# ekzhang/rpt

Measured on AMD Instinct MI355X. Metric: Msamples/s, higher is better.
Workload: dtype f64

## Files before the change

rpt_amd/csrc/api_render.cpp:

```cpp
#include "api_internal.h"

namespace rptapi {

int event_pair_begin(rptgpu_scene* h, int kind, bool on) {
  h->stats.kernel_launches[kind]++;
  if (!on || h->ev_used + 2 > MAX_EVENT_PAIRS * 2) return -1;
  while ((int)h->ev_pool.size() < h->ev_used + 2) {
    hipEvent_t e;
    HIP_TRY(hipEventCreate(&e));
    h->ev_pool.push_back(e);
  }
  const int e0 = h->ev_used;
  h->ev_used += 2;
  HIP_TRY(hipEventRecord(h->ev_pool[e0], h->stream));
  return e0;
}
void event_pair_end(rptgpu_scene* h, int kind, int e0) {
  if (e0 < 0) return;
  HIP_TRY(hipEventRecord(h->ev_pool[e0 + 1], h->stream));
  h->pending.push_back({kind, e0, e0 + 1});
}

struct Bracket {
  rptgpu_scene* h;
// ... 219 lines not shown
  tree_query(h, kt, ps, nullptr, n, -1, nullptr, nullptr, hook);
}
void query_visibility(rptgpu_scene* h, const KernelTable* kt, const rptdev::PathState& ps, int l, uint32_t n,
                      const uint32_t* d_n, const QueryHook* hook) {
  tree_query(h, kt, ps, h->shadow_q.p + (uint64_t)l * ps.cap, n, l, h->srt.p, d_n, hook);
}

rptdev::Camera make_camera(const RptCamera& c) {
  rptdev::Camera d{};
  std::memcpy(d.eye, c.eye, sizeof d.eye);
  std::memcpy(d.direction, c.direction, sizeof d.direction);
  std::memcpy(d.up, c.up, sizeof d.up);
  d.d = 1.0 / std::tan(c.fov / 2.0);
  const double* a = c.direction;
  const double* b = c.up;
  double cr[3] = {a[1] * b[2] - a[2] * b[1], a[2] * b[0] - a[0] * b[2], a[0] * b[1] - a[1] * b[0]};
  double len = std::sqrt((cr[0] * cr[0] + cr[1] * cr[1]) + cr[2] * cr[2]);
  for (int k = 0; k < 3; k++) d.right[k] = cr[k] / len;
  d.aperture = c.aperture;
  d.focal_distance = c.focal_distance;
  return d;
}

const char* bad_params(const RptRenderParams* p) {
  if (!p->width || !p->height || !p->iterations) return "width, height and iterations must be non-zero";
  if (p->max_bounces > 254) return "max_bounces > 254";
  if ((uint64_t)p->width * p->height >= (1ull << 31)) return "frame too large";
  if (p->part_count && p->part_index >= p->part_count) return "part_index >= part_count";
  if (p->precision_mode != RPT_PRECISION_F64_STRICT) return BAD_MODE;
  return nullptr;
}

int64_t free_memory() {
  size_t free_b = 0, total_b = 0;
  return hipMemGetInfo(&free_b, &total_b) == hipSuccess ? (int64_t)free_b : -1;
}

rptdev::PathState path_state(rptgpu_scene* h) {
  rptdev::PathState ps{};
  ps.ray = h->ray.p; ps.hit = h->hit.p; ps.hit_obj = h->hit_obj.p; ps.draw = h->draw.p;
  ps.pid = h->pid.p; ps.col = h->col.p;
  ps.ray_next = h->ray_next.p; ps.draw_next = h->draw_next.p; ps.pid_next = h->pid_next.p; ps.col_next = h->col_next.p;
  ps.rec = h->rec.p; ps.rec_parent = h->rec_parent.p; ps.last_col = h->last_col.p;
  ps.shadow = h->shadow.p; ps.cap = h->ws_cap; ps.rec_cap = h->ws_rec_cols;
  if (h->path_reorder) {
    ps.sort_keys = h->sort_kin.p; ps.sort_vals = h->sort_vin.p; ps.next_rows = h->next_rows.p;
    std::memcpy(ps.key_bounds, h->scene_bounds, sizeof ps.key_bounds);
  }
  return ps;
}

void render_persistent(rptgpu_scene* h, const KernelTable* kt, const RptRenderParams& p, rptdev::Frame fr,
                       const rptdev::Camera& cam, void* out, bool out_f32, bool packed, bool prof) {
  hipStream_t st = h->stream;
  const uint32_t npix = fr.npix;
  const bool print_launch = std::getenv("RPTGPU_PRINT_LAUNCH") != nullptr;
  const uint64_t lbuf_held = h->lbuf.n * sizeof(double);
  const int64_t free_b = lbuf_held < h->lbuf_max_bytes ? free_memory() : -1;
  const bool flat = h->all_flat && !h->dscene.force_general;
  FlatLayout lay = flat ? h->flat_layout : FlatLayout{};
  const uint32_t flat_lds = lay.off_end;
  if (RPT_PRETRACE_CULL && lay.pretrace_cull) {
    for (size_t i = 0; i < h->obj_geom.size() && i < 64 && lay.cull_n < (uint32_t)RPT_CULL_MAX; i++) {
      uint32_t r[4];
      if (((lay.cull_always >> i) & 1ull) ||
          !rpthost::pinhole_screen_rect(rpthost::world_box(h->obj_geom[i], h->top_insts[i]), cam, fr.width, fr.height, r))
        continue;
      lay.cull_obj[lay.cull_n] = (uint32_t)i;
      const bool off = r[0] > r[1] || r[2] > r[3];
      lay.cull_lo[lay.cull_n] = off ? 0xffffffffu : (r[0] | (r[2] << 16));
      lay.cull_ext[lay.cull_n] = off ? 0u : ((r[1] - r[0]) | ((r[3] - r[2]) << 16));
      lay.cull_n++;
    }
  }
  const rptplan::PersistentPlan pl = rptplan::plan_persistent(
      npix, p.iterations, p.max_bounces, h->num_cus, kt->paths_max_blocks_per_cu(flat ? &lay : nullptr, flat_lds, false),
      h->lbuf_max_bytes, lbuf_held, free_b, h->paths_chunk, h->all_flat, h->dscene.force_general, h->flat_layout.obj_filter);
  bool park = flat && h->opt.env_park != 0 && h->dscene.env_kind != RPT_ENV_COLOR;
  if (park && kt->paths_max_blocks_per_cu(&lay, flat_lds, true) < pl.per_cu) park = false;
  h->prec.alloc((uint64_t)rpt_fold_ring_slots(p.max_bounces) * rptdev::REC_FIELDS * ((uint64_t)pl.nblocks * 64));
  h->lbuf.alloc(std::max<uint64_t>(1, (uint64_t)pl.spp_l * 3 * npix));
  if (print_launch)
    std::fprintf(stderr, "rpt_paths<%s>: %d blocks/CU x %d CUs -> %u blocks, %u samples per work item, %u launch(es) of %u spp, "
                 "dynamic LDS %u B per wave (the flat scene's tables)%s%s%s\n",
                 flat ? (lay.obj_filter ? "KdFlatF" : lay.n_tris ? "KdFlat" : "KdFlatG") : "KdLds", pl.per_cu, h->num_cus, pl.nblocks,
                 pl.chunk, pl.n_launch, pl.spp_l, flat_lds, park ? " + parked environment lookups" : "",
                 flat && lay.n_tris && lay.fuse_query && !park ? ", shadow and bounce rays in one query" : "",
                 flat && lay.n_tris && lay.fuse_query && !park && lay.scene_consts ? ", a hit's scene constants from the wave's tables" : "");
  h->counters.alloc(4);
  h->pcounters.alloc(16);
  HIP_TRY(hipMemsetAsync(h->pcounters.p, 0, 16 * sizeof(unsigned long long), st));
  for (uint32_t s0 = 0; s0 < p.iterations; s0 += pl.spp_l) {
    const uint32_t spp = std::min(pl.spp_l, p.iterations - s0);
    const uint64_t items = rptplan::work_items(npix, spp, pl.chunk);
    fr.sample_base = p.sample_index_base + s0;
    HIP_TRY(hipMemsetAsync(h->counters.p, 0, sizeof(uint32_t), st));
    { Bracket b(h, RPT_K_PATHS, prof);
      kt->paths(st, h->dscene, fr, cam, h->counters.p, h->prec.p, h->pcounters.p, h->lbuf.p, spp, pl.chunk, (uint32_t)items,
                pl.nblocks, lay, flat, flat_lds, park, h->opt.paths_batch);
      b.done(); }
    kt->sum_samples(st, fr, h->lbuf.p, spp, s0 == 0);
    if (print_launch) {
      uint32_t ended = 0;
      HIP_TRY(hipMemcpyAsync(&ended, h->counters.p, sizeof ended, hipMemcpyDeviceToHost, st));
      HIP_TRY(hipStreamSynchronize(st));
      const uint32_t batch_used = h->opt.paths_batch ? std::min<uint32_t>(h->opt.paths_batch, RPT_PATHS_BATCH_MAX)
                                                      : std::min(256u, std::max((uint32_t)items / (std::max(1u, pl.nblocks) * 32u), 16u));
      std::fprintf(stderr, "rpt_paths work counter: ended at %u for %llu items; %u waves, claims of at most %u: dead claims %lld of at most %llu\n",
                   ended, (unsigned long long)items, pl.nblocks, batch_used, (long long)ended - (long long)items,
                   (unsigned long long)pl.nblocks * (64u + batch_used));
    }
  }
  HIP_TRY(hipGetLastError());
  kt->finish(st, fr, (double)p.iterations, std::pow(2.0, p.exposure_value), out, out_f32, packed);
  unsigned long long rc[16] = {0};
  HIP_TRY(hipMemcpyAsync(rc, h->pcounters.p, sizeof rc, hipMemcpyDeviceToHost, st));
  HIP_TRY(hipStreamSynchronize(st));
  if (std::getenv("RPTGPU_PRINT_PHASES")) print_prof(kt, "rpt_paths");
  h->stats.samples += (uint64_t)npix * p.iterations;
  h->stats.extend_rays += rc[0];
  h->stats.shadow_rays += rc[1];
  h->stats.shadow_rays_traced += rc[1];
}

bool run_pass(rptgpu_scene* h, const KernelTable* kt, const RptRenderParams& p, const rptdev::Frame& fr,
              const RaySource& src, uint32_t n_paths, uint32_t spp, bool prof, const QueryHook& qhook, uint64_t* cols) {
  hipStream_t st = h->stream;
  rptdev::PathState ps = path_state(h);
  const int nlights = h->dscene.num_lights;
  const uint32_t nctr = 2u + (uint32_t)nlights;
  HIP_TRY(hipMemsetAsync(h->counters.p, 0, 2 * (size_t)nctr * sizeof(uint32_t), st));
  uint32_t cset = 0;
  if (h->has_deep) reset_tree_counters(h);
  { Bracket b(h, RPT_K_RAYGEN, prof);
    if (src.cam) kt->raygen(st, fr, *src.cam, ps, n_paths);
    else kt->raygen_rays(st, fr, src.origins, src.dirs, src.first_draw, src.ids_out, src.id_base, ps, n_paths);
    b.done(); }
  h->stats.samples += n_paths;
  uint32_t n_active = n_paths;
  const uint32_t* const queue = nullptr;
  uint32_t* const next = nullptr;
  uint64_t rec_off = 0;
  const bool by_object = h->has_deep && (!(p.flags & RPT_FLAG_GENERAL_TRAVERSAL) || h->tree_kids);
  for (uint32_t depth = 0; depth <= p.max_bounces && n_active; depth++) {
    if (rec_off + n_active > h->ws_rec_cols) {
      *cols = rec_off + n_active;
      return false;
    }
    { Bracket b(h, RPT_K_EXTEND, prof);
      if (by_object)
        query_closest(h, kt, ps, n_active, &qhook);
      else
        kt->extend(st, h->dscene, ps, queue, n_active);
      b.done(); }
    h->stats.extend_rays += n_active;
    uint32_t* const ctrs = h->counters.p + (size_t)cset * nctr;
    uint32_t* const ctrs_next = h->counters.p + (size_t)(cset ^ 1u) * nctr;
    cset ^= 1u;
    { Bracket b(h, RPT_K_SHADE, prof);
      kt->shade(st, h->dscene, fr, ps, queue, n_active, depth, next, ctrs, h->shadow_q.p, ctrs_next, nctr, (uint32_t)rec_off); b.done(); }
    h->cnt_host.resize(2 + (size_t)nlights);
    uint32_t* cnt = h->cnt_host.data();
    HIP_TRY(hipMemcpyAsync(cnt, ctrs, (2 + (size_t)nlights) * sizeof(uint32_t), hipMemcpyDeviceToHost, st));
    HIP_TRY(hipStreamSynchronize(st));
    for (int l = 0; l < nlights; l++) h->stats.shadow_rays_traced += cnt[2 + l];
    if (prof && h->pending.size() >= 256) drain_events(h);
    h->stats.shadow_rays += (uint64_t)cnt[1] * (uint64_t)h->dscene.num_shadow_lights;
    if (nlights > 0) {
      Bracket b(h, RPT_K_SHADOW, prof);
      if (by_object) {
        for (int l = 0; l < nlights; l++)
// ... 226 lines not shown
```

rpt_amd/csrc/kernels.h:

```cpp
#pragma once
#include <hip/hip_runtime.h>
#include <stdint.h>

#include "device_types.h"
#include "launch_limits.h"

#ifndef RPT_FLAT_RUN
#define RPT_FLAT_RUN 6
#endif

#define RPT_PATHS_WAVE_LDS 20480u
#define RPT_PATHS_WALKER_LDS 2560u
#ifndef RPT_RAY_STASH
#define RPT_RAY_STASH 2
#endif
#ifndef RPT_FUSE_QUERY
#define RPT_FUSE_QUERY 1
#endif
#ifndef RPT_SHADE_SPLIT
#define RPT_SHADE_SPLIT 1
#endif
#ifndef RPT_PRETRACE_CULL
#define RPT_PRETRACE_CULL 1
#endif
#define RPT_CULL_MAX 4
#ifndef RPT_SCENE_CONSTS
#define RPT_SCENE_CONSTS 5
#endif
#define RPT_MAT_CONSTS_BYTES 88u
#define RPT_CUBE_NORMALS_BYTES 144u
#define RPT_PATHS_STASH_LDS 4864u
#define RPT_PATHS_STASH_HIT_LDS 6656u
#define RPT_PATHS_STASH_MAX_LDS (RPT_RAY_STASH >= 2 ? RPT_PATHS_STASH_HIT_LDS : RPT_PATHS_STASH_LDS)
#ifndef RPT_PARK_K
#define RPT_PARK_K 4
#endif
#define RPT_PATHS_PARK_LDS (RPT_PARK_K * 2624u)
#ifndef RPT_PATH_REORDER_MIN
#define RPT_PATH_REORDER_MIN (1u << 20)
#endif

#define RPT_RETIRE_ITEMS 16u
#define RPT_RETIRE_TILE (RPT_RETIRE_ITEMS * 256u)

struct FlatLayout {
  uint32_t off_tris, off_refs, off_mat, off_leaf;
  uint32_t off_end;
  uint32_t n_refs, n_tris;
  uint32_t off_qtab, plane_cnt;
  const double* plane_vals;
  uint32_t obj_filter;
  uint32_t off_obox;
  const rptdev::LeafBox* obj_box;
  const double* obj_grid;
  uint64_t obj_always;
  uint32_t fuse_query;
  uint32_t pretrace_cull, cull_n;
  uint64_t cull_always;
  uint32_t cull_obj[RPT_CULL_MAX], cull_lo[RPT_CULL_MAX], cull_ext[RPT_CULL_MAX];
  uint32_t scene_consts, off_consts;
};

struct SortBufs {
  uint32_t *keys_in, *keys_out, *vals_in;
  void* tmp;
  size_t tmp_bytes;
};

#ifndef RPT_TT_WAVES
#define RPT_TT_WAVES 4
#endif
#ifndef RPT_TT_LEVELS
#define RPT_TT_LEVELS 7
#endif
#define RPT_TT_LEVELS_MIN RPT_TT_LEVELS
struct GenericStack {
  double* defer;
  double* frame;
  uint32_t threads, levels, frames;
};
struct StackSpill {
  uint32_t* node;
  double* ts;
  double* bmax;
  uint32_t threads;
  uint32_t zeros_common;
  double* rays;
  GenericStack gen;
  uint32_t* gen_overflow;
  uint32_t gen_blocks_few, gen_blocks_all;
};

struct QueryHook {
  void (*mark)(void* ctx, int kind, int end);
  void* ctx;
};

struct QueryTuning {
  uint32_t ctr_set;
  uint32_t sort_min_rays;
};

struct KernelTable {
  void (*raygen)(hipStream_t, const rptdev::Frame&, const rptdev::Camera&, const rptdev::PathState&, uint32_t n_paths);
  void (*raygen_rays)(hipStream_t, const rptdev::Frame&, const double* origins, const double* dirs, uint32_t first_draw,
                      uint32_t* ids_out, uint32_t id_base, const rptdev::PathState&, uint32_t n_paths);
  void (*extend)(hipStream_t, const rptdev::Scene&, const rptdev::PathState&, const uint32_t* queue, uint32_t n);
  void (*extend_rays)(hipStream_t, const rptdev::Scene&, const double* o, const double* d, uint64_t n, double* out_t,
                      double* out_n, int32_t* out_obj);
  void (*shade)(hipStream_t, const rptdev::Scene&, const rptdev::Frame&, const rptdev::PathState&,
                const uint32_t* queue, uint32_t n, uint32_t depth, uint32_t* next_queue, uint32_t* counters, uint32_t* sq,
                uint32_t* zero_next , uint32_t zero_n,
                uint32_t rec_off );
  void (*shadow_rays)(hipStream_t, const rptdev::Scene&, const rptdev::PathState&, const uint32_t* sq_all,
                      const uint32_t* sq_counts, uint32_t n_max, int num_lights, double* srt);
// ... 44 lines not shown
```

rpt_amd/csrc/kernels/paths.inc:

```

#ifndef RPT_PARK_FLUSH
#define RPT_PARK_FLUSH 160
#endif
struct ParkLds {
  double d[RPT_PARK_K][3][64];
  uint32_t u[RPT_PARK_K][4][64];
  uint8_t list[RPT_PARK_K * 64];
};
static_assert(sizeof(ParkLds) == RPT_PATHS_PARK_LDS, "kernels.h sizes the wave's LDS budget with it");
static_assert(RPT_PARK_K >= 1 && RPT_PARK_K <= 4, "two bits for the entry in ParkLds::list, three for a lane's count");
struct PersistArgs {
  uint32_t* work_counter;
  double* rec;
  unsigned long long* ray_counters;
  double* lbuf;
  uint32_t spp;
  uint32_t chunk;
  uint32_t n_items;
  uint32_t nthreads;
  uint32_t ring;
  uint32_t batch;
  uint32_t park_off;
  FlatLayout flat;
};
// ... 73 lines not shown
}
RPT_DEV void path_ended(const PersistArgs& pa, const Frame& fr, double* __restrict__ rec, double (*fold_l)[64],
                        uint32_t (*fold_u)[64], uint32_t lane, uint32_t& fold_st, const D3& A, uint32_t depth, uint32_t b,
                        uint32_t s, uint32_t p_local) {
  if (depth == 0) {
    double* lb = pa.lbuf + (uint64_t)s * 3 * fr.npix + p_local;
    lb[0] = A.x;
    lb[fr.npix] = A.y;
    lb[2 * (uint64_t)fr.npix] = A.z;
  } else if ((fold_st & 0xffffu) == 0u) {
    fold_l[0][lane] = A.x; fold_l[1][lane] = A.y; fold_l[2][lane] = A.z;
    fold_u[0][lane] = depth; fold_u[1][lane] = b; fold_u[2][lane] = s; fold_u[3][lane] = p_local;
    fold_st |= depth;
  } else {
    double* r = rec + b * REC_FIELDS;
    r[0] = A.x; r[1] = A.y; r[2] = A.z;
    r[3] = __longlong_as_double((long long)((uint64_t)s | ((uint64_t)p_local << 32)));
    r[4] = __longlong_as_double((long long)depth);
  }
}
RPT_DEV void park_push(ParkLds& park, uint32_t lane, uint32_t& pcnt, uint32_t& park_hd, uint32_t& park_recs, uint32_t& fold_st,
                       uint32_t ring, const D3& d, uint32_t depth, uint32_t s, uint32_t p_local) {
  const uint32_t k = pcnt, b = fold_st >> 16;
  park.d[k][0][lane] = d.x; park.d[k][1][lane] = d.y; park.d[k][2][lane] = d.z;
  park.u[k][0][lane] = depth; park.u[k][1][lane] = b; park.u[k][2][lane] = s; park.u[k][3][lane] = p_local;
  if (depth != 0u) {
    if (park_hd == 0xffffffffu) park_hd = b;
    park_recs += depth;
    fold_st = (fold_st & 0xffffu) | (next_header_slot(b, depth, ring) << 16);
  }
  pcnt = k + 1u;
}
struct RayStash {
  double v[7][64];
  uint32_t u[5][64];
};
static_assert(sizeof(RayStash) == RPT_PATHS_STASH_LDS, "kernels.h sizes the wave's LDS budget with it");
struct RayStashHit {
  double v[10][64];
  uint32_t u[6][64];
};
static_assert(sizeof(RayStashHit) == RPT_PATHS_STASH_HIT_LDS, "kernels.h sizes the wave's LDS budget with it");
template <class S> RPT_DEV void stash_put_pos(S& st, uint32_t lane, const D3& o) {
  st.v[0][lane] = o.x; st.v[1][lane] = o.y; st.v[2][lane] = o.z;
}
template <class S> RPT_DEV void stash_put_dir(S& st, uint32_t lane, const D3& d) {
  st.v[3][lane] = d.x; st.v[4][lane] = d.y; st.v[5][lane] = d.z;
}
template <class S> RPT_DEV void stash_put_ray(S& st, uint32_t lane, const D3& o, const D3& d) {
  stash_put_pos(st, lane, o);
  stash_put_dir(st, lane, d);
}
template <class S> RPT_DEV void stash_take_ray(const S& st, uint32_t lane, D3& o, D3& d) {
  o = mk(st.v[0][lane], st.v[1][lane], st.v[2][lane]);
  d = mk(st.v[3][lane], st.v[4][lane], st.v[5][lane]);
}
template <class S> RPT_DEV void stash_swap_ray(S& st, uint32_t lane, D3& o, D3& d) {
  D3 so, sd;
  stash_take_ray(st, lane, so, sd);
  stash_put_ray(st, lane, o, d);
  o = so; d = sd;
}
template <class S> RPT_DEV void stash_put_path(S& st, uint32_t lane, uint32_t p_local, uint32_t pixel, uint32_t s, uint32_t s_end, const Rng& r) {
  st.v[6][lane] = __longlong_as_double((long long)r.hi);
  st.u[0][lane] = p_local; st.u[1][lane] = pixel; st.u[2][lane] = s; st.u[3][lane] = s_end;
  st.u[4][lane] = r.draw;
}
template <class S> RPT_DEV void stash_take_path(const S& st, uint32_t lane, const Frame& fr, uint32_t& p_local, uint32_t& pixel, uint32_t& s,
                             uint32_t& s_end, Rng& r) {
  p_local = st.u[0][lane]; pixel = st.u[1][lane]; s = st.u[2][lane]; s_end = st.u[3][lane];
  r = rng_make(fr.seed, pixel, fr.sample_base + s, 0);
  r.draw = st.u[4][lane];
  r.hi = (uint64_t)__double_as_longlong(st.v[6][lane]);
}
RPT_DEV void stash_put_hit(RayStashHit& st, uint32_t lane, const D3& pos, const D3& nrm, int obj) {
  stash_put_pos(st, lane, pos);
  st.v[7][lane] = nrm.x; st.v[8][lane] = nrm.y; st.v[9][lane] = nrm.z;
  st.u[5][lane] = (uint32_t)obj;
}
RPT_DEV void stash_take_hit(const RayStashHit& st, uint32_t lane, D3& pos, D3& d, D3& nrm, int& obj) {
  stash_take_ray(st, lane, pos, d);
  nrm = mk(st.v[7][lane], st.v[8][lane], st.v[9][lane]);
  obj = (int)st.u[5][lane];
}
#ifndef RPT_STASH_REFILL_MIN
#define RPT_STASH_REFILL_MIN 32
#endif
RPT_DEV void end_path(const PersistArgs& pa, const Frame& fr, double* __restrict__ rec, double (*fold_l)[64],
                      uint32_t (*fold_u)[64], uint32_t lane, uint32_t& fold_st, uint32_t ring, const D3& A, uint32_t depth,
                      uint32_t s, uint32_t p_local) {
  const uint32_t b = fold_st >> 16;
  path_ended(pa, fr, rec, fold_l, fold_u, lane, fold_st, A, depth, b, s, p_local);
  if (depth != 0u) fold_st = (fold_st & 0xffffu) | (next_header_slot(b, depth, ring) << 16);
}
template <bool PARK>
RPT_DEV void walker_step(const PersistArgs& pa, const Frame& fr, const double* __restrict__ rec, double (*fold_l)[64],
                         uint32_t (*fold_u)[64], uint32_t lane, uint32_t& fold_st, uint32_t ring, uint32_t park_hd,
                         double probe_chk ) {
  const uint32_t wk = fold_st & 0xffffu, cb = fold_st >> 16;
  const uint32_t wD = fold_u[0][lane], wb = fold_u[1][lane];
  uint32_t pos = wb + wk;
  if (pos >= ring) pos -= ring;
  const uint32_t nh = next_header_slot(wb, wD, ring);
  const bool last = wk == 1u, more = last && nh != cb && (!PARK || nh != park_hd);
  double v[REC_FIELDS], hd[5] = {0.0, 0.0, 0.0, 0.0, 0.0};
#ifdef RPT_PROBE_NO_RING
  (void)pos;
#pragma unroll
  for (int q = 0; q < REC_FIELDS; q++) v[q] = probe_chk * (double)(q + 1);
#else
  {
    const double* r = rec + pos * REC_FIELDS;
#pragma unroll
    for (int q = 0; q < REC_FIELDS; q++) v[q] = r[q];
  }
#endif
  if (more) {
    const double* r = rec + nh * REC_FIELDS;
#pragma unroll
    for (int q = 0; q < 5; q++) hd[q] = r[q];
  }
  D3 L = mk(fold_l[0][lane], fold_l[1][lane], fold_l[2][lane]);
  D3 Ak = mk(v[0], v[1], v[2]);
  D3 f = mk(v[3], v[4], v[5]);
  D3 indirect = v[6] * cmul(f, L) * v[7];
  L = mk(Ak.x + fmin(indirect.x, FIREFLY_CLAMP), Ak.y + fmin(indirect.y, FIREFLY_CLAMP),
         Ak.z + fmin(indirect.z, FIREFLY_CLAMP));
  if (!last) {
    fold_l[0][lane] = L.x; fold_l[1][lane] = L.y; fold_l[2][lane] = L.z;
    fold_st -= 1u;
  } else {
    double* lb = pa.lbuf + (uint64_t)fold_u[2][lane] * 3 * fr.npix + fold_u[3][lane];
    lb[0] = L.x;
    lb[fr.npix] = L.y;
    lb[2 * (uint64_t)fr.npix] = L.z;
    uint32_t nk = 0u;
    if (more) {
      const uint64_t sp = (uint64_t)__double_as_longlong(hd[3]);
      nk = (uint32_t)__double_as_longlong(hd[4]);
      fold_l[0][lane] = hd[0]; fold_l[1][lane] = hd[1]; fold_l[2][lane] = hd[2];
      fold_u[0][lane] = nk; fold_u[1][lane] = nh; fold_u[2][lane] = (uint32_t)sp; fold_u[3][lane] = (uint32_t)(sp >> 32);
    }
    fold_st = (cb << 16) | nk;
  }
}
template <class LDS, bool PARK ,
          bool FUSE = false ,
          bool CONSTS = false >
__global__ void __launch_bounds__(64, RPT_PATHS_WAVES) rpt_paths(Scene sc, Frame fr, Camera cam, PersistArgs pa) {
  extern __shared__ __attribute__((aligned(16))) unsigned char flat_smem[];
  __shared__ typename PathsLds<LDS>::type kd_store;
  LDS* kd_ldsp = reinterpret_cast<LDS*>(&kd_store);
  constexpr bool FILTERED = std::is_same<LDS, KdFlatF>::value;
  constexpr bool IS_FLAT = std::is_same<LDS, KdFlat>::value || std::is_same<LDS, KdFlatG>::value || FILTERED;
  constexpr bool TRIS_IN_LDS = std::is_same<LDS, KdFlat>::value;
  FlatLds fl{};
  if constexpr (IS_FLAT) {
    const FlatLayout& lay = pa.flat;
    const uint32_t l = threadIdx.x;
    TriX* l_lrec = reinterpret_cast<TriX*>(flat_smem);
    Tri* l_tris = reinterpret_cast<Tri*>(flat_smem + lay.off_tris);
    uint32_t* l_refs = reinterpret_cast<uint32_t*>(flat_smem + lay.off_refs);
    Material* l_mat = reinterpret_cast<Material*>(flat_smem + lay.off_mat);
    uint32_t(*l_leaf)[4] = reinterpret_cast<uint32_t(*)[4]>(flat_smem + lay.off_leaf);
    const double* src = reinterpret_cast<const double*>(sc.lrec);
    double* dst = reinterpret_cast<double*>(l_lrec);
    for (uint32_t i = l; i < lay.n_refs * (uint32_t)(sizeof(TriX) / 8); i += 64) dst[i] = src[i];
    if constexpr (TRIS_IN_LDS) {
      src = reinterpret_cast<const double*>(sc.tris);
      dst = reinterpret_cast<double*>(l_tris);
      for (uint32_t i = l; i < lay.n_tris * (uint32_t)(sizeof(Tri) / 8); i += 64) dst[i] = src[i];
    }
    for (uint32_t i = l; i < lay.n_refs; i += 64) l_refs[i] = sc.refs[i];
    for (uint32_t i = l; i < (uint32_t)sc.num_objects * (uint32_t)(sizeof(Material) / 8); i += 64) {
      uint32_t ob = i / (uint32_t)(sizeof(Material) / 8), w = i - ob * (uint32_t)(sizeof(Material) / 8);
      reinterpret_cast<double*>(l_mat)[i] = reinterpret_cast<const double*>(sc.materials + sc.insts[ob].material)[w];
    }
    for (uint32_t ob = l; ob < (uint32_t)sc.num_objects; ob += 64) {
      const Inst& in = sc.insts[ob];
      uint32_t e0 = 0, e1 = 0, e2 = 0, e3 = 0;
      if (in.kind == RPT_SHAPE_MESH) {
        const Tree& tr = sc.trees[in.tree];
        e0 = tr.ref_base; e1 = tr.prim_base; e2 = tr.root_first; e3 = tr.root_leaf - 1u;
      }
      l_leaf[ob][0] = e0; l_leaf[ob][1] = e1; l_leaf[ob][2] = e2; l_leaf[ob][3] = e3;
      if constexpr (FILTERED) {
        l_leaf[ob][3] = e3 | ((uint32_t)in.kind << 8) | (in.has_xf ? 1u << 16 : 0u);
        double* ob6 = reinterpret_cast<double*>(flat_smem + lay.off_obox) + 6u * ob;
        for (int k = 0; k < 6; k++) ob6[k] = in.bounds[k];
      }
    }
    if constexpr (CONSTS) {
      static_assert(FUSE, "the tables serve the fused form");
      scene_consts_fill(sc, sc.tris, l, flat_smem + lay.off_consts);
      fl.consts = flat_smem + lay.off_consts;
    }
    __syncthreads();
    sc.lrec = l_lrec;
    if constexpr (TRIS_IN_LDS) sc.tris = l_tris;
    sc.refs = l_refs;
    fl.lrec = l_lrec; fl.tris = sc.tris; fl.refs = l_refs; fl.obj_mat = l_mat; fl.obj_leaf = l_leaf;
    fl.qtab = reinterpret_cast<double*>(flat_smem + lay.off_qtab);
    fl.plane_vals = lay.plane_vals;
    fl.plane_cnt = lay.plane_cnt;
    if constexpr (FILTERED) {
      fl.obox = reinterpret_cast<const double*>(flat_smem + lay.off_obox);
      fl.obj_box = lay.obj_box; fl.obj_grid = lay.obj_grid; fl.obj_always = lay.obj_always;
    }
  }
  const uint32_t tid = blockIdx.x * blockDim.x + threadIdx.x;
  const uint32_t lane = __lane_id();
  double* __restrict__ rec = pa.rec + (uint64_t)tid * pa.ring * REC_FIELDS;
  __shared__ double fold_l[3][64];
  __shared__ uint32_t fold_u[4][64];
  uint32_t fold_st = 0;
  const uint32_t ring = pa.ring;
  uint32_t p_local = 0, pixel = 0, s = 0, s_end = 0, depth = 0;
  bool done = false, in_path = false;
  D3 o = mk(0, 0, 0), d = mk(0, 0, 1);
  Rng rng = rng_make(fr.seed, 0, 0, 0);
  uint32_t n_ext = 0, n_sh = 0;
#ifdef RPT_PROBE_NO_RING
  double probe_chk = 0.0;
#else
  constexpr double probe_chk = 0.0;
#endif
  const double dim = (double)max(fr.width, fr.height);
  constexpr bool STASH = RPT_RAY_STASH && std::is_same<LDS, KdFlat>::value;
  constexpr bool PRETRACE = STASH && RPT_RAY_STASH >= 2 && !PARK;
  static_assert(!FUSE || PRETRACE, "the fused form is a form of the pre-traced kernel");
  using StashT = typename std::conditional<PRETRACE, RayStashHit, RayStash>::type;
  __shared__ typename std::conditional<STASH, StashT, int>::type stash_store;
  auto& stash = *reinterpret_cast<StashT*>(&stash_store);
  bool stash_valid = false, exhausted = false;
  bool pend = false;
#if RPT_PRETRACE_CULL
  uint32_t near = ~0u;
#endif
  ItemPool pool{0u, 0u, 0u};
  constexpr bool park_on = PARK;
  ParkLds& park = *reinterpret_cast<ParkLds*>(flat_smem + (park_on ? pa.park_off : 0u));
  uint32_t pcnt = 0, park_hd = 0xffffffffu, park_recs = 0;
  D3 nx_pos = mk(0, 0, 0), nx_nrm = mk(0, 0, 0);
  int nx_obj = -1;
  PROF_INIT();

  for (;;) {
    if constexpr (STASH) {
      bool refill = __ballot(!in_path && !stash_valid && !exhausted) != 0ull;
      if constexpr (PRETRACE) refill = refill || __popcll(__ballot(!stash_valid && !exhausted)) >= RPT_STASH_REFILL_MIN;
      if (refill) {
        const bool gen = !stash_valid && !exhausted;
        uint32_t g_p_local = p_local, g_pixel = pixel, g_s = s + (in_path ? 1u : 0u), g_s_end = s_end;
        const bool want_item = gen && g_s >= g_s_end;
        const bool got = fetch_item(pa, fr, lane, want_item, pool, g_p_local, g_pixel, g_s, g_s_end);
        if (want_item && !got) exhausted = true;
        PROF_PHASE(PF_P_FETCH);
        if (gen && !exhausted) {
          D3 go, gd;
          Rng gr;
          camera_ray(fr, cam, dim, g_pixel, g_s, go, gd, gr);
#if RPT_PRETRACE_CULL
          if constexpr (FUSE) near = cull_near(pa.flat, g_pixel, fr.width);
#endif
          stash_put_ray(stash, lane, go, gd);
          stash_put_path(stash, lane, g_p_local, g_pixel, g_s, g_s_end, gr);
          stash_valid = true;
          pend = PRETRACE;
        }
        PROF_PHASE(PF_P_RAYGEN);
      }
      if (!PRETRACE && !in_path && stash_valid) {
        stash_take_ray(stash, lane, o, d);
        stash_take_path(stash, lane, fr, p_local, pixel, s, s_end, rng);
        stash_valid = false;
        depth = 0;
        in_path = true;
      }
      done = !in_path && exhausted && !(PRETRACE && stash_valid);
      if (__ballot(!done || (fold_st & 0xffffu) != 0u || pcnt != 0u) == 0) break;
    } else {
      const bool need = !done && !in_path && s == s_end;
      if (!fetch_item(pa, fr, lane, need, pool, p_local, pixel, s, s_end) && need) done = true;
      if (__ballot(!done || (fold_st & 0xffffu) != 0u || pcnt != 0u) == 0) break;
      PROF_PHASE(PF_P_FETCH);
      if (!done && !in_path) {
        uint32_t y = pixel / fr.width, x = pixel - y * fr.width;
        double xn = ((double)(2 * x + 1) - (double)fr.width) / dim;
        double yn = ((double)(2 * (fr.height - y) - 1) - (double)fr.height) / dim;
        rng = rng_make(fr.seed, pixel, fr.sample_base + s, 0);
        double dx = gen_range(rng, -1.0 / dim, 1.0 / dim);
        double dy = gen_range(rng, -1.0 / dim, 1.0 / dim);
        double px = xn + dx, py = yn + dy;
        D3 direction = ld3(cam.direction), up = ld3(cam.up), right = ld3(cam.right);
        o = ld3(cam.eye);
        D3 new_dir = cam.d * direction + px * right + py * up;
        if (cam.aperture > 0.0) {
          D3 focal_point = o + normalize(new_dir) * cam.focal_distance;
          double a, b;
          unit_disc(rng, a, b);
          o = o + (a * right + b * up) * cam.aperture;
          new_dir = focal_point - o;
        }
        d = normalize(new_dir);
        depth = 0;
        in_path = true;
      }
    }

    PROF_PHASE(PF_P_RAYGEN);
    bool ending = false, esc = false;
    D3 A_end = mk(0, 0, 0);
    D3 h_pos = mk(0, 0, 0), h_nrm = mk(0, 0, 0);
    int h_obj = -1;
    if constexpr (FUSE) {
      h_pos = nx_pos; h_nrm = nx_nrm; h_obj = nx_obj;
      nx_pos = mk(0, 0, 0); nx_nrm = mk(0, 0, 0); nx_obj = -1;
      if (__ballot(pend) != 0ull) {
        if (pend) {
          D3 so, sd;
          stash_take_ray(stash, lane, so, sd);
          double t = INF;
          D3 hn = mk(0, 0, 0);
#if RPT_PRETRACE_CULL
          const uint64_t skip = cull_skip_mask(pa.flat, near);
          PROF_COUNT(PF_P_PRETRACE);
          const int ho = flat_query<false, true, CONSTS>(sc, &fl, so, sd, -INF, t, hn, skip);
#else
          const int ho = flat_query<false, false, CONSTS>(sc, &fl, so, sd, -INF, t, hn);
#endif
          n_ext++;
          if (ho < 0) hn = env_color(sc, sd);
          stash_put_hit(stash, lane, so + t * sd, hn, ho);
          pend = false;
        }
      }
    } else if constexpr (PRETRACE) {
#pragma unroll 1
      for (uint32_t pass = __ballot(pend && in_path) != 0ull ? 0u : 1u; pass < 2u; pass++) {
        const bool pre = pend, run = pend || (pass == 1u && in_path);
        if (pre) stash_swap_ray(stash, lane, o, d);
        double t = INF;
        h_nrm = mk(0, 0, 0);
        h_obj = -1;
        if (run) {
          h_obj = flat_query<false>(sc, &fl, o, d, -INF, t, h_nrm);
          n_ext++;
          if (h_obj < 0) h_nrm = env_color(sc, d);
        }
        h_pos = o + t * d;
        if (pre) {
          D3 ro, rd;
          stash_take_ray(stash, lane, ro, rd);
          stash_put_dir(stash, lane, d);
          stash_put_hit(stash, lane, h_pos, h_nrm, h_obj);
          o = ro; d = rd;
          pend = false;
        }
      }
    }
    if constexpr (PRETRACE) {
      PROF_PHASE(PF_P_HIT);
      if (in_path && h_obj < 0 && stash_valid) {
        end_path(pa, fr, rec, fold_l, fold_u, lane, fold_st, ring, h_nrm, depth, s, p_local);
        in_path = false;
      }
      if (!in_path && stash_valid) {
        stash_take_hit(stash, lane, h_pos, d, h_nrm, h_obj);
        stash_take_path(stash, lane, fr, p_local, pixel, s, s_end, rng);
        stash_valid = false;
        depth = 0;
        in_path = true;
      }
      PROF_PHASE(PF_P_RAYGEN);
    }
    if constexpr (FUSE) {
      if (in_path && h_obj < 0) {
        PROF_PHASE(PF_P_ILLUM);
        ending = true;
        A_end = h_nrm;
      } else if (in_path) {
        const D3 world_pos = h_pos, nrm = h_nrm;
        const Material& mat = fl.obj_mat[h_obj];
        const D3 wo = -normalize(d);
        const D3 color = mat.emittance * ld3(mat.color);
        D3 wl, lt, wi;
        double dist;
        bool cont;
#if RPT_SHADE_SPLIT
        CLight& lg = clight(sc, 0);
        CInst& li = cinst(sc, lg.inst);
        if (lg.kind == RPT_LIGHT_OBJECT && li.kind == RPT_SHAPE_MESH && !li.has_xf && __ballot(mat.transparent != 0) == 0ull) {
          CTree& tr = ctree(sc, li.tree);
          constexpr bool CM = CONSTS && SC_MAT, CL = CONSTS && SC_LIGHT;
          const MatConsts* mcs = CM ? mat_consts_of(&fl, h_obj) : nullptr;
          double fs;
          if constexpr (CM) {
            fs = mcs->fs;
          } else {
            const D3 mc = ld3(mat.color);
            const double f0 = pow2((mat.index - 1.0) / (mat.index + 1.0));
            const double mean = ((mc.x + mc.y) + mc.z) / 3.0;
            fs = (1.0 - mat.metallic) * f0 + mat.metallic * mean;
            fs = fs * (1.0 - 0.2) + 1.0 * 0.2;
          }
          cont = depth < fr.max_bounces;
          HitDraws dr;
          hit_draws<CM>(rng, cont, tr.num_prims, tr.sample_zone, fs, dr, mcs);
          n_sh++;
          PROF_PHASE(PF_P_DRAWS);
          D3 intensity;
          illuminate_mesh<CL>(lg, tr, sc.tris + tr.prim_base + dr.tri, world_pos, dr, intensity, wl, dist,
                              CL ? light_pdf_of(sc, &fl) : nullptr);
          double pdf;
          sample_f_opaque<CM>(mat, nrm, wo, fs, dr, wi, pdf, mcs);
          lt = mk(0, 0, 0) + cmul(bsdf_opaque<CM>(mat, nrm, wo, wl, mcs), intensity) * dot(wl, nrm);
          const D3 f = bsdf_opaque<CM>(mat, nrm, wo, wi, mcs);
          PROF_PHASE(PF_P_SHADE);
          if (cont) {
            rec_store_bsdf(rec + rec_slot(fold_st, depth, ring) * REC_FIELDS, f, 1.0 / pdf, fabs(dot(wi, nrm)));
          } else {
            wi = wl;
          }
          PROF_PHASE(PF_P_RECORD);
        } else
#endif
        {
        D3 intensity;
        illuminate(sc, clight(sc, 0), world_pos, rng, intensity, wl, dist);
        n_sh++;
        PROF_PHASE(PF_P_ILLUM);
        lt = mk(0, 0, 0) + cmul(bsdf(mat, nrm, wo, wl), intensity) * dot(wl, nrm);
        PROF_PHASE(PF_P_NEE);
        wi = wl;
        double pdf = 1.0;
        cont = depth < fr.max_bounces && sample_f(mat, nrm, wo, rng, wi, pdf);
        PROF_PHASE(PF_P_SAMPLE);
        if (cont) {
          const D3 f = bsdf(mat, nrm, wo, wi);
          PROF_PHASE(PF_P_BSDF);
          rec_store_bsdf(rec + rec_slot(fold_st, depth, ring) * REC_FIELDS, f, 1.0 / pdf, fabs(dot(wi, nrm)));
          PROF_PHASE(PF_P_RECORD);
        }
        }
// ... 208 lines not shown
```

Before: 1463.

## Replace per-lane pre-trace stash with a wave-level pool of pre-traced hits

In the fused flat-scene path kernel, the per-lane ray stash is replaced by a 64-slot LDS ring buffer shared by the wave. Camera rays are generated and traced in bulk whenever the pool drops below a refill mark, and lanes whose path ended pop ready hits by rank. The aim is to keep lanes busy with fewer divergent single-lane refills and to batch primary-ray traversal. It adds ballots, a __syncthreads per refill and different loop termination logic, which risks divergence and synchronisation overhead. The default RPT_SCENE_CONSTS also changes from 5 to 7.

Measured after the change: 1645, median of 6. 1.12x the previous value.

```diff
diff --git a/rpt_amd/csrc/api_render.cpp b/rpt_amd/csrc/api_render.cpp
--- a/rpt_amd/csrc/api_render.cpp
+++ b/rpt_amd/csrc/api_render.cpp
@@ -325,11 +325,12 @@
   h->lbuf.alloc(std::max<uint64_t>(1, (uint64_t)pl.spp_l * 3 * npix));
   if (print_launch)
     std::fprintf(stderr, "rpt_paths<%s>: %d blocks/CU x %d CUs -> %u blocks, %u samples per work item, %u launch(es) of %u spp, "
-                 "dynamic LDS %u B per wave (the flat scene's tables)%s%s%s\n",
+                 "dynamic LDS %u B per wave (the flat scene's tables)%s%s%s%s\n",
                  flat ? (lay.obj_filter ? "KdFlatF" : lay.n_tris ? "KdFlat" : "KdFlatG") : "KdLds", pl.per_cu, h->num_cus, pl.nblocks,
                  pl.chunk, pl.n_launch, pl.spp_l, flat_lds, park ? " + parked environment lookups" : "",
                  flat && lay.n_tris && lay.fuse_query && !park ? ", shadow and bounce rays in one query" : "",
-                 flat && lay.n_tris && lay.fuse_query && !park && lay.scene_consts ? ", a hit's scene constants from the wave's tables" : "");
+                 flat && lay.n_tris && lay.fuse_query && !park && lay.scene_consts ? ", a hit's scene constants from the wave's tables" : "",
+                 RPT_HIT_POOL && flat && lay.n_tris && lay.fuse_query && !park ? ", pre-traced hits in a wave-level pool" : "");
   h->counters.alloc(4);
   h->pcounters.alloc(16);
   HIP_TRY(hipMemsetAsync(h->pcounters.p, 0, 16 * sizeof(unsigned long long), st));
diff --git a/rpt_amd/csrc/hit_pool.h b/rpt_amd/csrc/hit_pool.h
--- /dev/null
+++ b/rpt_amd/csrc/hit_pool.h
@@ -0,0 +1,24 @@
+#pragma once
+#include <stdint.h>
+
+#if defined(__HIPCC__) || defined(__CUDACC__)
+#define RPT_POOL_FN __host__ __device__ static inline
+#else
+#define RPT_POOL_FN static inline
+#endif
+
+RPT_POOL_FN uint32_t rpt_pool_slot(uint32_t head, uint32_t k, uint32_t cap) { return (head + k) % cap; }
+RPT_POOL_FN uint32_t rpt_pool_rank(uint64_t mask, uint32_t lane) {
+  return (uint32_t)__builtin_popcountll(mask & ((1ull << lane) - 1ull));
+}
+RPT_POOL_FN bool rpt_pool_pop_ok(uint32_t r, uint32_t count) { return r < count; }
+RPT_POOL_FN uint32_t rpt_pool_gen_limit(uint32_t count, uint32_t cap) { return cap - count; }
+RPT_POOL_FN void rpt_pool_after_pop(uint32_t& head, uint32_t& count, uint64_t pop_mask, uint32_t cap) {
+  const uint32_t want = (uint32_t)__builtin_popcountll(pop_mask), n = want < count ? want : count;
+  head = (head + n) % cap;
+  count -= n;
+}
+RPT_POOL_FN void rpt_pool_after_push(uint32_t& count, uint64_t push_mask) { count += (uint32_t)__builtin_popcountll(push_mask); }
+RPT_POOL_FN bool rpt_pool_refill(uint32_t count, uint32_t n_need, uint32_t cap, uint32_t refill_min) {
+  return count + refill_min <= cap || count < n_need;
+}
diff --git a/rpt_amd/csrc/kernels.h b/rpt_amd/csrc/kernels.h
--- a/rpt_amd/csrc/kernels.h
+++ b/rpt_amd/csrc/kernels.h
@@ -3,6 +3,7 @@
 #include <stdint.h>
 
 #include "device_types.h"
+#include "hit_pool.h"
 #include "launch_limits.h"
 
 #ifndef RPT_FLAT_RUN
@@ -25,12 +26,25 @@
 #endif
 #define RPT_CULL_MAX 4
 #ifndef RPT_SCENE_CONSTS
-#define RPT_SCENE_CONSTS 5
+#define RPT_SCENE_CONSTS 7
 #endif
 #define RPT_MAT_CONSTS_BYTES 88u
 #define RPT_CUBE_NORMALS_BYTES 144u
 #define RPT_PATHS_STASH_LDS 4864u
 #define RPT_PATHS_STASH_HIT_LDS 6656u
+#ifndef RPT_HIT_POOL
+#define RPT_HIT_POOL 1
+#endif
+#ifndef RPT_POOL_CAP
+#define RPT_POOL_CAP 64u
+#endif
+#ifndef RPT_POOL_REFILL
+#define RPT_POOL_REFILL 56u
+#endif
+#define RPT_PATHS_POOL_LDS (RPT_POOL_CAP * 100u)
+static_assert(RPT_POOL_CAP >= 64u && RPT_POOL_REFILL >= 1u && RPT_POOL_REFILL <= RPT_POOL_CAP,
+              "a refill of 64 lanes has to fit an empty pool, and a full pool has to fall to the refill mark");
+static_assert(RPT_PATHS_POOL_LDS <= RPT_PATHS_STASH_HIT_LDS, "the host's fit checks leave room for RayStashHit only");
 #define RPT_PATHS_STASH_MAX_LDS (RPT_RAY_STASH >= 2 ? RPT_PATHS_STASH_HIT_LDS : RPT_PATHS_STASH_LDS)
 #ifndef RPT_PARK_K
 #define RPT_PARK_K 4
diff --git a/rpt_amd/csrc/kernels/paths.inc b/rpt_amd/csrc/kernels/paths.inc
--- a/rpt_amd/csrc/kernels/paths.inc
+++ b/rpt_amd/csrc/kernels/paths.inc
@@ -179,6 +179,29 @@
   stash_take_ray(st, lane, pos, d);
   nrm = mk(st.v[7][lane], st.v[8][lane], st.v[9][lane]);
   obj = (int)st.u[5][lane];
+}
+struct HitPool {
+  double v[10][RPT_POOL_CAP];
+  uint32_t u[5][RPT_POOL_CAP];
+};
+static_assert(sizeof(HitPool) == RPT_PATHS_POOL_LDS, "kernels.h sizes the wave's LDS budget with it");
+RPT_DEV void pool_put(HitPool& hp, uint32_t slot, const D3& pos, const D3& d, const D3& nrm, int obj, uint32_t p_local,
+                      uint32_t pixel, uint32_t s, const Rng& r) {
+  hp.v[0][slot] = pos.x; hp.v[1][slot] = pos.y; hp.v[2][slot] = pos.z;
+  hp.v[3][slot] = d.x; hp.v[4][slot] = d.y; hp.v[5][slot] = d.z;
+  hp.v[6][slot] = __longlong_as_double((long long)r.hi);
+  hp.v[7][slot] = nrm.x; hp.v[8][slot] = nrm.y; hp.v[9][slot] = nrm.z;
+  hp.u[0][slot] = (uint32_t)obj; hp.u[1][slot] = p_local; hp.u[2][slot] = pixel; hp.u[3][slot] = s; hp.u[4][slot] = r.draw;
+}
+RPT_DEV void pool_take(const HitPool& hp, uint32_t slot, const Frame& fr, D3& pos, D3& d, D3& nrm, int& obj, uint32_t& p_local,
+                       uint32_t& s, Rng& r) {
+  pos = mk(hp.v[0][slot], hp.v[1][slot], hp.v[2][slot]);
+  d = mk(hp.v[3][slot], hp.v[4][slot], hp.v[5][slot]);
+  nrm = mk(hp.v[7][slot], hp.v[8][slot], hp.v[9][slot]);
+  obj = (int)hp.u[0][slot]; p_local = hp.u[1][slot]; s = hp.u[3][slot];
+  r = rng_make(fr.seed, hp.u[2][slot], fr.sample_base + s, 0);
+  r.draw = hp.u[4][slot];
+  r.hi = (uint64_t)__double_as_longlong(hp.v[6][slot]);
 }
 #ifndef RPT_STASH_REFILL_MIN
 #define RPT_STASH_REFILL_MIN 32
@@ -326,9 +349,13 @@
   constexpr bool STASH = RPT_RAY_STASH && std::is_same<LDS, KdFlat>::value;
   constexpr bool PRETRACE = STASH && RPT_RAY_STASH >= 2 && !PARK;
   static_assert(!FUSE || PRETRACE, "the fused form is a form of the pre-traced kernel");
-  using StashT = typename std::conditional<PRETRACE, RayStashHit, RayStash>::type;
+  constexpr bool POOL = FUSE && RPT_HIT_POOL != 0;
+  using StashT = typename std::conditional<POOL, HitPool, typename std::conditional<PRETRACE, RayStashHit, RayStash>::type>::type;
   __shared__ typename std::conditional<STASH, StashT, int>::type stash_store;
   auto& stash = *reinterpret_cast<StashT*>(&stash_store);
+  struct PoolState { uint32_t g_p_local = 0, g_s = ~0u; uint32_t head = 0, cnt = 0; };
+  struct NoPoolState {};
+  [[maybe_unused]] typename std::conditional<POOL, PoolState, NoPoolState>::type ps;
   bool stash_valid = false, exhausted = false;
   bool pend = false;
 #if RPT_PRETRACE_CULL
@@ -343,7 +370,47 @@
   PROF_INIT();
 
   for (;;) {
-    if constexpr (STASH) {
+    if constexpr (POOL) {
+      const uint32_t n_need = (uint32_t)__popcll(__ballot(!in_path || nx_obj < 0));
+      const uint64_t work_mask = __ballot(!exhausted);
+      if (work_mask != 0ull && rpt_pool_refill(ps.cnt, n_need, RPT_POOL_CAP, RPT_POOL_REFILL)) {
+        const bool turn = !exhausted && rpt_pool_rank(work_mask, lane) < rpt_pool_gen_limit(ps.cnt, RPT_POOL_CAP);
+        const bool want_item = turn && ps.g_s == ~0u;
+        uint32_t f_pixel = 0, f_s_end = 0;
+        const bool got = fetch_item(pa, fr, lane, want_item, pool, ps.g_p_local, f_pixel, ps.g_s, f_s_end);
+        if (want_item && !got) exhausted = true;
+        PROF_PHASE(PF_P_FETCH);
+        const bool gen = turn && !exhausted;
+        const uint64_t gen_mask = __ballot(gen);
+        if (gen) {
+          const uint32_t g_pixel = fr.pixels[ps.g_p_local];
+          D3 go, gd;
+          Rng gr;
+          camera_ray(fr, cam, dim, g_pixel, ps.g_s, go, gd, gr);
+          PROF_PHASE(PF_P_RAYGEN);
+          double t = INF;
+          D3 hn = mk(0, 0, 0);
+#if RPT_PRETRACE_CULL
+          const uint64_t skip = cull_skip_mask(pa.flat, cull_near(pa.flat, g_pixel, fr.width));
+          PROF_COUNT(PF_P_PRETRACE);
+          const int ho = flat_query<false, true, CONSTS>(sc, &fl, go, gd, -INF, t, hn, skip);
+#else
+          const int ho = flat_query<false, false, CONSTS>(sc, &fl, go, gd, -INF, t, hn);
+#endif
+          n_ext++;
+          if (ho < 0) hn = env_color(sc, gd);
+          pool_put(stash, rpt_pool_slot(ps.head, ps.cnt + rpt_pool_rank(gen_mask, lane), RPT_POOL_CAP), go + t * gd, gd, hn, ho,
+                   ps.g_p_local, g_pixel, ps.g_s, gr);
+          ps.g_s++;
+          if (ps.g_s % pa.chunk == 0u || ps.g_s == pa.spp) ps.g_s = ~0u;
+          PROF_PHASE(PF_P_HIT);
+        }
+        rpt_pool_after_push(ps.cnt, gen_mask);
+        __syncthreads();
+      }
+      done = !in_path && exhausted;
+      if (ps.cnt == 0u && __ballot(!done || (fold_st & 0xffffu) != 0u) == 0) break;
+    } else if constexpr (STASH) {
       bool refill = __ballot(!in_path && !stash_valid && !exhausted) != 0ull;
       if constexpr (PRETRACE) refill = refill || __popcll(__ballot(!stash_valid && !exhausted)) >= RPT_STASH_REFILL_MIN;
       if (refill) {
@@ -413,23 +480,25 @@
     if constexpr (FUSE) {
       h_pos = nx_pos; h_nrm = nx_nrm; h_obj = nx_obj;
       nx_pos = mk(0, 0, 0); nx_nrm = mk(0, 0, 0); nx_obj = -1;
-      if (__ballot(pend) != 0ull) {
-        if (pend) {
-          D3 so, sd;
-          stash_take_ray(stash, lane, so, sd);
-          double t = INF;
-          D3 hn = mk(0, 0, 0);
+      if constexpr (!POOL) {
+        if (__ballot(pend) != 0ull) {
+          if (pend) {
+            D3 so, sd;
+            stash_take_ray(stash, lane, so, sd);
+            double t = INF;
+            D3 hn = mk(0, 0, 0);
 #if RPT_PRETRACE_CULL
-          const uint64_t skip = cull_skip_mask(pa.flat, near);
-          PROF_COUNT(PF_P_PRETRACE);
-          const int ho = flat_query<false, true, CONSTS>(sc, &fl, so, sd, -INF, t, hn, skip);
+            const uint64_t skip = cull_skip_mask(pa.flat, near);
+            PROF_COUNT(PF_P_PRETRACE);
+            const int ho = flat_query<false, true, CONSTS>(sc, &fl, so, sd, -INF, t, hn, skip);
 #else
-          const int ho = flat_query<false, false, CONSTS>(sc, &fl, so, sd, -INF, t, hn);
-#endif
-          n_ext++;
-          if (ho < 0) hn = env_color(sc, sd);
-          stash_put_hit(stash, lane, so + t * sd, hn, ho);
-          pend = false;
+            const int ho = flat_query<false, false, CONSTS>(sc, &fl, so, sd, -INF, t, hn);
+#endif
+            n_ext++;
+            if (ho < 0) hn = env_color(sc, sd);
+            stash_put_hit(stash, lane, so + t * sd, hn, ho);
+            pend = false;
+          }
         }
       }
     } else if constexpr (PRETRACE) {
@@ -456,7 +525,19 @@
         }
       }
     }
-    if constexpr (PRETRACE) {
+    if constexpr (POOL) {
+      PROF_PHASE(PF_P_HIT);
+      const bool need = !in_path || h_obj < 0;
+      const uint64_t need_mask = __ballot(need);
+      if (need && rpt_pool_pop_ok(rpt_pool_rank(need_mask, lane), ps.cnt)) {
+        if (in_path) end_path(pa, fr, rec, fold_l, fold_u, lane, fold_st, ring, h_nrm, depth, s, p_local);
+        pool_take(stash, rpt_pool_slot(ps.head, rpt_pool_rank(need_mask, lane), RPT_POOL_CAP), fr, h_pos, d, h_nrm, h_obj, p_local, s, rng);
+        depth = 0;
+        in_path = true;
+      }
+      rpt_pool_after_pop(ps.head, ps.cnt, need_mask, RPT_POOL_CAP);
+      PROF_PHASE(PF_P_RAYGEN);
+    } else if constexpr (PRETRACE) {
       PROF_PHASE(PF_P_HIT);
       if (in_path && h_obj < 0 && stash_valid) {
         end_path(pa, fr, rec, fold_l, fold_u, lane, fold_st, ring, h_nrm, depth, s, p_local);
```
